# ZrrSkywalker/MonoDETR

Hardware: NVIDIA H100
Metric: images/sec (1280x384, fwd+bwd) (higher is better)
Workload: dtype f32 (BF16x3: error-compensated bf16 tensor-core products, fp32 accumulate)

## Files before the change

### monodetr_b200/csrc/attention.cu

```cuda
#include <cuda_runtime.h>
#include <math.h>
#include <stdint.h>

#include "../../include/monodetr_b200.h"
#include "launch.cuh"
#include "rng.cuh"
#include "tc_common.cuh"

namespace {

using namespace mdb;

constexpr int HD = 32;
constexpr int BR = 64;
constexpr int BC = 64;
constexpr int kTileBytes = BC * HD * 4;
constexpr int ATT_THREADS = 128;

struct AttnParams {
    const float *q, *k, *v;
    const uint8_t* kpm;
    float* out;
    float* lse;
    int B, H, Lq, Lk, ldq, ldk, ldv, ldo;
    float scale;
    float drop_p;
    const unsigned long long* seed;
    unsigned long long site;
    const float *dout, *o;
    float* delta;
    float *dq, *dk, *dv;
    int lddq, lddk, lddv;
};

__device__ __forceinline__ uint32_t f2tf32(float x) {
    uint32_t r;
    asm("cvt.rna.tf32.f32 %0, %1;" : "=r"(r) : "f"(x));
    return r;
}
__device__ __forceinline__ void split_tf32(float x, uint32_t& hi, uint32_t& lo) {
    hi = f2tf32(x);
    lo = f2tf32(x - __uint_as_float(hi));
}
struct AFrag {
    uint32_t hi[4][4];
    uint32_t lo[4][4];
};
__device__ __forceinline__ void load_afrag(AFrag& f, const float* base, int ld, int r0, int nrows, int lane, float mul) {
    const int g = lane >> 2, t = lane & 3;
    const int ra = r0 + g, rb = r0 + g + 8;
    const float* pa = base + (size_t)min(ra, nrows - 1) * ld;
    const float* pb = base + (size_t)min(rb, nrows - 1) * ld;
    const float ma = ra < nrows ? mul : 0.f, mb = rb < nrows ? mul : 0.f;
#pragma unroll
    for (int ks = 0; ks < 4; ++ks) {
        split_tf32(pa[ks * 8 + t] * ma, f.hi[ks][0], f.lo[ks][0]);
        split_tf32(pb[ks * 8 + t] * mb, f.hi[ks][1], f.lo[ks][1]);
        split_tf32(pa[ks * 8 + t + 4] * ma, f.hi[ks][2], f.lo[ks][2]);
        split_tf32(pb[ks * 8 + t + 4] * mb, f.hi[ks][3], f.lo[ks][3]);
    }
}

__device__ __forceinline__ uint32_t nt_off(int r, int c) { return (uint32_t)(r * 128 + ((((c >> 2) ^ (r & 7))) << 4) + (c & 3) * 4); }
__device__ __forceinline__ uint32_t nn_off(int r, int c) {
    const int kk = r & 31, q = kk & 7;
    const int kpos = (kk & ~7) + ((q & 1) ? 4 + (q >> 1) : (q >> 1));
    return (uint32_t)((r >> 5) * 4096 + c * 128 + ((((kpos >> 2) ^ (c & 7))) << 4) + (kpos & 3) * 4);
}

template <int NS>
__device__ __forceinline__ void gemm_nt(float (&c)[8][4], const AFrag& a, uint32_t th, uint32_t tl) {
    float (&d)[32] = reinterpret_cast<float (&)[32]>(c);
#pragma unroll
    for (int i = 0; i < 32; ++i) d[i] = 0.f;
    wgmma_fence();
#pragma unroll
    for (int ks = 0; ks < 4; ++ks) {
        const uint64_t bh = make_wgmma_desc_sw128(th + ks * 32);
        if (NS == 3) {
            const uint64_t bl = make_wgmma_desc_sw128(tl + ks * 32);
            wgmma_tf32_n64(d, a.lo[ks], bh, 1);
            wgmma_tf32_n64(d, a.hi[ks], bl, 1);
        }
        wgmma_tf32_n64(d, a.hi[ks], bh, 1);
    }
    wgmma_commit();
    wgmma_wait_all();
    wgmma_fence_operands(d);
}

template <int NS>
__device__ __forceinline__ void gemm_nn(float (&acc)[4][4], const float (&p)[8][4], uint32_t th, uint32_t tl) {
    float (&d)[16] = reinterpret_cast<float (&)[16]>(acc);
#pragma unroll
    for (int half = 0; half < 2; ++half) {
        uint32_t ah[4][4], al[4][4];
#pragma unroll
        for (int u = 0; u < 4; ++u) {
            const int kt = half * 4 + u;
            split_tf32(p[kt][0], ah[u][0], al[u][0]);
            split_tf32(p[kt][2], ah[u][1], al[u][1]);
            split_tf32(p[kt][1], ah[u][2], al[u][2]);
            split_tf32(p[kt][3], ah[u][3], al[u][3]);
        }
        wgmma_fence();
#pragma unroll
        for (int u = 0; u < 4; ++u) {
            const uint32_t off = half * 4096 + u * 32;
            const uint64_t bh = make_wgmma_desc_sw128(th + off);
            if (NS == 3) {
                const uint64_t bl = make_wgmma_desc_sw128(tl + off);
                wgmma_tf32_n32(d, al[u], bh, 1);
                wgmma_tf32_n32(d, ah[u], bl, 1);
            }
            wgmma_tf32_n32(d, ah[u], bh, 1);
        }
        wgmma_commit();
        wgmma_wait_all();
        wgmma_fence_operands(d);
    }
}

constexpr int STG = BC * HD;
__device__ __forceinline__ void stage_tile(float* stg, const float* base, int ld, int r0, int nrows) {
#pragma unroll
    for (int u = 0; u < 4; ++u) {
        const int i = threadIdx.x + u * ATT_THREADS;
        const int r = i >> 3, c = (i & 7) * 4;
        const bool ok = r0 + r < nrows;
        const float* src = ok ? base + ((size_t)(r0 + r) * ld + c) : base;
        const uint32_t dst = (uint32_t)__cvta_generic_to_shared(stg) + (uint32_t)i * 16u;
        const int nbytes = ok ? 16 : 0;
        asm volatile("cp.async.cg.shared.global [%0], [%1], 16, %2;" ::"r"(dst), "l"(src), "r"(nbytes) : "memory");
    }
}
__device__ __forceinline__ void stage_commit() { asm volatile("cp.async.commit_group;" ::: "memory"); }
__device__ __forceinline__ void stage_wait() { asm volatile("cp.async.wait_all;" ::: "memory"); }
__device__ __forceinline__ void unstage_tile(uint8_t* nt_hi, uint8_t* nt_lo, uint8_t* nn_hi, uint8_t* nn_lo, const float* stg) {
#pragma unroll
    for (int u = 0; u < 4; ++u) {
        const int i = threadIdx.x + u * ATT_THREADS;
        const int r = i >> 3, c = (i & 7) * 4;
        const float4 v = *reinterpret_cast<const float4*>(stg + i * 4);
        uint32_t h[4], l[4];
        split_tf32(v.x, h[0], l[0]); split_tf32(v.y, h[1], l[1]); split_tf32(v.z, h[2], l[2]); split_tf32(v.w, h[3], l[3]);
        if (nt_hi) *reinterpret_cast<uint4*>(nt_hi + nt_off(r, c)) = make_uint4(h[0], h[1], h[2], h[3]);
        if (nt_lo) *reinterpret_cast<uint4*>(nt_lo + nt_off(r, c)) = make_uint4(l[0], l[1], l[2], l[3]);
#pragma unroll
        for (int e = 0; e < 4; ++e) {
            if (nn_hi) *reinterpret_cast<uint32_t*>(nn_hi + nn_off(r, c + e)) = h[e];
            if (nn_lo) *reinterpret_cast<uint32_t*>(nn_lo + nn_off(r, c + e)) = l[e];
        }
    }
}
static_assert(BC * (HD / 4) == 4 * ATT_THREADS, "tile loader mapping");

__device__ __forceinline__ float quad_max(float v) {
    v = fmaxf(v, __shfl_xor_sync(0xffffffffu, v, 1));
    return fmaxf(v, __shfl_xor_sync(0xffffffffu, v, 2));
}
__device__ __forceinline__ float quad_sum(float v) {
    v += __shfl_xor_sync(0xffffffffu, v, 1);
    return v + __shfl_xor_sync(0xffffffffu, v, 2);
}

struct DropCtx {
    uint32_t key, thr;
    float inv_keep;
    bool on;
};
__device__ __forceinline__ DropCtx make_drop(const AttnParams& p, int b, int h) {
    DropCtx d;
    d.on = p.drop_p > 0.f;
    d.inv_keep = 1.f / (1.f - p.drop_p);
    d.thr = mdb::rng_thr16(p.drop_p);
    d.key = 0u;
    if (d.on) d.key = mdb::rng_key32(*p.seed + p.site * 0x9E3779B97F4A7C15ull, (unsigned long long)(b * p.H + h));
    return d;
}
__device__ __forceinline__ float keep_scale(const DropCtx& d, uint32_t row_base, int j) {
    return mdb::rng_keep16(d.key, row_base + (uint32_t)j, d.thr) ? d.inv_keep : 0.f;
}

__device__ __forceinline__ uint32_t fetch_dead(const AttnParams& p, int b, int k0) {
    const int j = k0 + (int)threadIdx.x;
    if (threadIdx.x >= BC) return 0u;
    if (j >= p.Lk) return 1u;
    return (p.kpm && p.kpm[(size_t)b * p.Lk + j]) ? 1u : 0u;
}

__global__ void __launch_bounds__(ATT_THREADS, 3)
attn_fwd_kernel(const AttnParams p) {
    extern __shared__ __align__(1024) uint8_t dyn_smem[];
    uint8_t* sKh = dyn_smem;
    uint8_t* sKl = sKh + kTileBytes;
    uint8_t* sVh = sKl + kTileBytes;
    uint8_t* sVl = sVh + kTileBytes;
    float* gK = reinterpret_cast<float*>(sVl + kTileBytes);
    float* gV = gK + STG;
    uint8_t* sDead = reinterpret_cast<uint8_t*>(gV + STG);
    const int b = blockIdx.z, h = blockIdx.y;
    const int warp = threadIdx.x >> 5, lane = threadIdx.x & 31;
    const int g = lane >> 2, t = lane & 3;
    const int r0 = blockIdx.x * BR + warp * 16;
    const float* qb = p.q + (size_t)b * p.Lq * p.ldq + h * HD;
    const float* kb = p.k + (size_t)b * p.Lk * p.ldk + h * HD;
    const float* vb = p.v + (size_t)b * p.Lk * p.ldv + h * HD;
    const DropCtx drop = make_drop(p, b, h);
    stage_tile(gK, kb, p.ldk, 0, p.Lk);
    stage_tile(gV, vb, p.ldv, 0, p.Lk);
    stage_commit();
    uint32_t ndead = fetch_dead(p, b, 0);
    AFrag qa;
    load_afrag(qa, qb, p.ldq, r0, p.Lq, lane, p.scale);
    float acc[4][4];
#pragma unroll
    for (int i = 0; i < 4; ++i) acc[i][0] = acc[i][1] = acc[i][2] = acc[i][3] = 0.f;
    float m0 = -INFINITY, m1 = -INFINITY, l0 = 0.f, l1 = 0.f;
    const int qi0 = r0 + g, qi1 = r0 + g + 8;
    const uint32_t rb0 = (uint32_t)qi0 * (uint32_t)p.Lk, rb1 = (uint32_t)qi1 * (uint32_t)p.Lk;

    for (int k0 = 0; k0 < p.Lk; k0 += BC) {
        stage_wait();
        __syncthreads();
        unstage_tile(sKh, sKl, nullptr, nullptr, gK);
        unstage_tile(nullptr, nullptr, sVh, sVl, gV);
        if (threadIdx.x < BC) sDead[threadIdx.x] = (uint8_t)ndead;
        mdb::fence_proxy_async_smem();
        __syncthreads();
        if (k0 + BC < p.Lk) {
            stage_tile(gK, kb, p.ldk, k0 + BC, p.Lk);
            stage_tile(gV, vb, p.ldv, k0 + BC, p.Lk);
            stage_commit();
            ndead = fetch_dead(p, b, k0 + BC);
        }
        float s[8][4];
        gemm_nt<3>(s, qa, mdb::smem_u32(sKh), mdb::smem_u32(sKl));
        float mx0 = -INFINITY, mx1 = -INFINITY;
#pragma unroll
        for (int nt = 0; nt < 8; ++nt) {
            const uchar2 dd = *reinterpret_cast<const uchar2*>(&sDead[nt * 8 + 2 * t]);
            if (dd.x) { s[nt][0] = -INFINITY; s[nt][2] = -INFINITY; }
            if (dd.y) { s[nt][1] = -INFINITY; s[nt][3] = -INFINITY; }
            mx0 = fmaxf(mx0, fmaxf(s[nt][0], s[nt][1]));
            mx1 = fmaxf(mx1, fmaxf(s[nt][2], s[nt][3]));
        }
        const float mn0 = fmaxf(m0, quad_max(mx0)), mn1 = fmaxf(m1, quad_max(mx1));
        const float c0 = (mn0 == -INFINITY) ? 1.f : __expf(m0 - mn0), c1 = (mn1 == -INFINITY) ? 1.f : __expf(m1 - mn1);
        l0 *= c0; l1 *= c1;
#pragma unroll
        for (int dn = 0; dn < 4; ++dn) { acc[dn][0] *= c0; acc[dn][1] *= c0; acc[dn][2] *= c1; acc[dn][3] *= c1; }
#pragma unroll
        for (int nt = 0; nt < 8; ++nt) {
#pragma unroll
            for (int e = 0; e < 2; ++e) {
                const int j = k0 + nt * 8 + 2 * t + e;
                float p0 = (mn0 == -INFINITY) ? 0.f : __expf(s[nt][e] - mn0);
                float p1 = (mn1 == -INFINITY) ? 0.f : __expf(s[nt][2 + e] - mn1);
                l0 += p0; l1 += p1;
                if (drop.on) {
                    p0 *= keep_scale(drop, rb0, j);
                    p1 *= keep_scale(drop, rb1, j);
                }
                s[nt][e] = p0; s[nt][2 + e] = p1;
            }
        }
        m0 = mn0; m1 = mn1;
        gemm_nn<3>(acc, s, mdb::smem_u32(sVh), mdb::smem_u32(sVl));
    }
    l0 = quad_sum(l0); l1 = quad_sum(l1);
    const float i0 = l0 > 0.f ? 1.f / l0 : 0.f, i1 = l1 > 0.f ? 1.f / l1 : 0.f;
    float* ob = p.out + (size_t)b * p.Lq * p.ldo + h * HD;
#pragma unroll
    for (int dn = 0; dn < 4; ++dn) {
        if (qi0 < p.Lq) *reinterpret_cast<float2*>(ob + (size_t)qi0 * p.ldo + dn * 8 + 2 * t) = make_float2(acc[dn][0] * i0, acc[dn][1] * i0);
        if (qi1 < p.Lq) *reinterpret_cast<float2*>(ob + (size_t)qi1 * p.ldo + dn * 8 + 2 * t) = make_float2(acc[dn][2] * i1, acc[dn][3] * i1);
    }
    if (t == 0) {
        float* lp = p.lse + ((size_t)b * p.H + h) * p.Lq;
        if (qi0 < p.Lq) lp[qi0] = l0 > 0.f ? m0 + __logf(l0) : -INFINITY;
        if (qi1 < p.Lq) lp[qi1] = l1 > 0.f ? m1 + __logf(l1) : -INFINITY;
    }
}

__global__ void attn_delta_kernel(const AttnParams p) {
    const long long idx = blockIdx.x * (long long)blockDim.x + threadIdx.x;
    const long long n = (long long)p.B * p.Lq * p.H;
    if (idx >= n) return;
    const int h = (int)(idx % p.H);
    const long long bi = idx / p.H;
    const int i = (int)(bi % p.Lq);
    const int b = (int)(bi / p.Lq);
    const float* a = p.dout + (size_t)bi * p.ldo + h * HD;
    const float* o = p.o + (size_t)bi * p.ldo + h * HD;
    float s = 0.f;
#pragma unroll
    for (int d = 0; d < HD; d += 4) {
        const float4 x = *reinterpret_cast<const float4*>(a + d);
        const float4 y = *reinterpret_cast<const float4*>(o + d);
        s += x.x * y.x + x.y * y.y + x.z * y.z + x.w * y.w;
    }
    p.delta[((size_t)b * p.H + h) * p.Lq + i] = s;
}

__global__ void __launch_bounds__(ATT_THREADS, 3)
attn_bwd_dq_kernel(const AttnParams p) {
    extern __shared__ __align__(1024) uint8_t dyn_smem[];
    uint8_t* sKh = dyn_smem;
    uint8_t* sKl = sKh + kTileBytes;
    uint8_t* sKn = sKl + kTileBytes;
    uint8_t* sVh = sKn + kTileBytes;
    float* gK = reinterpret_cast<float*>(sVh + kTileBytes);
    float* gV = gK + STG;
    uint8_t* sDead = reinterpret_cast<uint8_t*>(gV + STG);
    const int b = blockIdx.z, h = blockIdx.y;
    const int warp = threadIdx.x >> 5, lane = threadIdx.x & 31;
    const int g = lane >> 2, t = lane & 3;
    const int r0 = blockIdx.x * BR + warp * 16;
    const float* qb = p.q + (size_t)b * p.Lq * p.ldq + h * HD;
    const float* gb = p.dout + (size_t)b * p.Lq * p.ldo + h * HD;
    const float* kb = p.k + (size_t)b * p.Lk * p.ldk + h * HD;
    const float* vb = p.v + (size_t)b * p.Lk * p.ldv + h * HD;
    const DropCtx drop = make_drop(p, b, h);
    stage_tile(gK, kb, p.ldk, 0, p.Lk);
    stage_tile(gV, vb, p.ldv, 0, p.Lk);
    stage_commit();
    uint32_t ndead = fetch_dead(p, b, 0);
    AFrag qa, ga;
    load_afrag(qa, qb, p.ldq, r0, p.Lq, lane, p.scale);
    load_afrag(ga, gb, p.ldo, r0, p.Lq, lane, 1.f);
    const int qi0 = r0 + g, qi1 = r0 + g + 8;
    const uint32_t rb0 = (uint32_t)qi0 * (uint32_t)p.Lk, rb1 = (uint32_t)qi1 * (uint32_t)p.Lk;
    const size_t st = ((size_t)b * p.H + h) * p.Lq;
    float lse0 = qi0 < p.Lq ? p.lse[st + qi0] : INFINITY, lse1 = qi1 < p.Lq ? p.lse[st + qi1] : INFINITY;
    if (lse0 == -INFINITY) lse0 = INFINITY;
    if (lse1 == -INFINITY) lse1 = INFINITY;
    const float dl0 = qi0 < p.Lq ? p.delta[st + qi0] : 0.f, dl1 = qi1 < p.Lq ? p.delta[st + qi1] : 0.f;
    float acc[4][4];
#pragma unroll
    for (int i = 0; i < 4; ++i) acc[i][0] = acc[i][1] = acc[i][2] = acc[i][3] = 0.f;

    for (int k0 = 0; k0 < p.Lk; k0 += BC) {
        stage_wait();
        __syncthreads();
        unstage_tile(sKh, sKl, sKn, nullptr, gK);
        unstage_tile(sVh, nullptr, nullptr, nullptr, gV);
        if (threadIdx.x < BC) sDead[threadIdx.x] = (uint8_t)ndead;
        mdb::fence_proxy_async_smem();
        __syncthreads();
        if (k0 + BC < p.Lk) {
            stage_tile(gK, kb, p.ldk, k0 + BC, p.Lk);
            stage_tile(gV, vb, p.ldv, k0 + BC, p.Lk);
            stage_commit();
            ndead = fetch_dead(p, b, k0 + BC);
        }
        float s[8][4], dp[8][4];
        gemm_nt<3>(s, qa, mdb::smem_u32(sKh), mdb::smem_u32(sKl));
        gemm_nt<1>(dp, ga, mdb::smem_u32(sVh), 0u);
#pragma unroll
        for (int nt = 0; nt < 8; ++nt) {
            const uchar2 dd = *reinterpret_cast<const uchar2*>(&sDead[nt * 8 + 2 * t]);
#pragma unroll
            for (int e = 0; e < 2; ++e) {
                const int j = k0 + nt * 8 + 2 * t + e;
                const bool dead = e ? dd.y : dd.x;
                float p0 = dead ? 0.f : __expf(s[nt][e] - lse0);
                float p1 = dead ? 0.f : __expf(s[nt][2 + e] - lse1);
                float d0 = dp[nt][e], d1 = dp[nt][2 + e];
                if (drop.on) {
                    d0 *= keep_scale(drop, rb0, j);
                    d1 *= keep_scale(drop, rb1, j);
                }
                s[nt][e] = p0 * (d0 - dl0);
                s[nt][2 + e] = p1 * (d1 - dl1);
            }
        }
        gemm_nn<1>(acc, s, mdb::smem_u32(sKn), 0u);
    }
    float* ob = p.dq + (size_t)b * p.Lq * p.lddq + h * HD;
#pragma unroll
    for (int dn = 0; dn < 4; ++dn) {
        if (qi0 < p.Lq) *reinterpret_cast<float2*>(ob + (size_t)qi0 * p.lddq + dn * 8 + 2 * t) = make_float2(acc[dn][0] * p.scale, acc[dn][1] * p.scale);
        if (qi1 < p.Lq) *reinterpret_cast<float2*>(ob + (size_t)qi1 * p.lddq + dn * 8 + 2 * t) = make_float2(acc[dn][2] * p.scale, acc[dn][3] * p.scale);
    }
}

__global__ void __launch_bounds__(ATT_THREADS, 2)
attn_bwd_dkv_kernel(const AttnParams p) {
    extern __shared__ __align__(1024) uint8_t dyn_smem[];
    uint8_t* sQh = dyn_smem;
    uint8_t* sQl = sQh + kTileBytes;
    uint8_t* sQn = sQl + kTileBytes;
    uint8_t* sGh = sQn + kTileBytes;
    uint8_t* sGn = sGh + kTileBytes;
    float* gQ = reinterpret_cast<float*>(sGn + kTileBytes);
    float* gG = gQ + STG;
    float* sL = gG + STG;
    float* sD = sL + BC;
    const int b = blockIdx.z, h = blockIdx.y;
    const int warp = threadIdx.x >> 5, lane = threadIdx.x & 31;
    const int g = lane >> 2, t = lane & 3;
    const int r0 = blockIdx.x * BR + warp * 16;
    const float* qb = p.q + (size_t)b * p.Lq * p.ldq + h * HD;
    const float* gb = p.dout + (size_t)b * p.Lq * p.ldo + h * HD;
    const float* kb = p.k + (size_t)b * p.Lk * p.ldk + h * HD;
    const float* vb = p.v + (size_t)b * p.Lk * p.ldv + h * HD;
    const DropCtx drop = make_drop(p, b, h);
    const size_t st = ((size_t)b * p.H + h) * p.Lq;
    auto fetch_stats = [&](int q0, float& l, float& d) {
        const int i = q0 + (int)threadIdx.x;
        l = INFINITY; d = 0.f;
        if (threadIdx.x < BC && i < p.Lq) {
            l = p.lse[st + i];
            d = p.delta[st + i];
            if (l == -INFINITY) l = INFINITY;
        }
    };
    float nl, nd;
    stage_tile(gQ, qb, p.ldq, 0, p.Lq);
    stage_tile(gG, gb, p.ldo, 0, p.Lq);
    stage_commit();
    fetch_stats(0, nl, nd);
    AFrag ka, va;
    load_afrag(ka, kb, p.ldk, r0, p.Lk, lane, p.scale);
    load_afrag(va, vb, p.ldv, r0, p.Lk, lane, 1.f);
    const int kj0 = r0 + g, kj1 = r0 + g + 8;
    const bool dead0 = kj0 >= p.Lk || (p.kpm && p.kpm[(size_t)b * p.Lk + min(kj0, p.Lk - 1)]);
    const bool dead1 = kj1 >= p.Lk || (p.kpm && p.kpm[(size_t)b * p.Lk + min(kj1, p.Lk - 1)]);
    float dk[4][4], dv[4][4];
#pragma unroll
    for (int i = 0; i < 4; ++i) {
        dk[i][0] = dk[i][1] = dk[i][2] = dk[i][3] = 0.f;
        dv[i][0] = dv[i][1] = dv[i][2] = dv[i][3] = 0.f;
    }

    for (int q0 = 0; q0 < p.Lq; q0 += BC) {
        stage_wait();
        __syncthreads();
        unstage_tile(sQh, sQl, sQn, nullptr, gQ);
        unstage_tile(sGh, nullptr, sGn, nullptr, gG);
        if (threadIdx.x < BC) { sL[threadIdx.x] = nl; sD[threadIdx.x] = nd; }
        mdb::fence_proxy_async_smem();
        __syncthreads();
        if (q0 + BC < p.Lq) {
            stage_tile(gQ, qb, p.ldq, q0 + BC, p.Lq);
            stage_tile(gG, gb, p.ldo, q0 + BC, p.Lq);
            stage_commit();
            fetch_stats(q0 + BC, nl, nd);
        }
        float s[8][4], dp[8][4];
        gemm_nt<3>(s, ka, mdb::smem_u32(sQh), mdb::smem_u32(sQl));
        gemm_nt<1>(dp, va, mdb::smem_u32(sGh), 0u);
        float pd[8][4];
#pragma unroll
        for (int nt = 0; nt < 8; ++nt) {
            const float2 l2 = *reinterpret_cast<const float2*>(&sL[nt * 8 + 2 * t]);
            const float2 d2 = *reinterpret_cast<const float2*>(&sD[nt * 8 + 2 * t]);
#pragma unroll
            for (int e = 0; e < 2; ++e) {
                const int i = q0 + nt * 8 + 2 * t + e;
                const float lse = e ? l2.y : l2.x, dl = e ? d2.y : d2.x;
                float p0 = dead0 ? 0.f : __expf(s[nt][e] - lse);
                float p1 = dead1 ? 0.f : __expf(s[nt][2 + e] - lse);
                float d0 = dp[nt][e], d1 = dp[nt][2 + e];
                float w0 = p0, w1 = p1;
                if (drop.on) {
                    const uint32_t rb = (uint32_t)i * (uint32_t)p.Lk;
                    const float k0s = keep_scale(drop, rb, kj0), k1s = keep_scale(drop, rb, kj1);
                    w0 *= k0s; w1 *= k1s; d0 *= k0s; d1 *= k1s;
                }
                pd[nt][e] = w0; pd[nt][2 + e] = w1;
                s[nt][e] = p0 * (d0 - dl);
                s[nt][2 + e] = p1 * (d1 - dl);
            }
        }
        gemm_nn<1>(dv, pd, mdb::smem_u32(sGn), 0u);
        gemm_nn<1>(dk, s, mdb::smem_u32(sQn), 0u);
    }
    float* dkb = p.dk + (size_t)b * p.Lk * p.lddk + h * HD;
    float* dvb = p.dv + (size_t)b * p.Lk * p.lddv + h * HD;
#pragma unroll
    for (int dn = 0; dn < 4; ++dn) {
        if (kj0 < p.Lk) {
            *reinterpret_cast<float2*>(dkb + (size_t)kj0 * p.lddk + dn * 8 + 2 * t) = make_float2(dk[dn][0] * p.scale, dk[dn][1] * p.scale);
            *reinterpret_cast<float2*>(dvb + (size_t)kj0 * p.lddv + dn * 8 + 2 * t) = make_float2(dv[dn][0], dv[dn][1]);
        }
        if (kj1 < p.Lk) {
            *reinterpret_cast<float2*>(dkb + (size_t)kj1 * p.lddk + dn * 8 + 2 * t) = make_float2(dk[dn][2] * p.scale, dk[dn][3] * p.scale);
            *reinterpret_cast<float2*>(dvb + (size_t)kj1 * p.lddv + dn * 8 + 2 * t) = make_float2(dv[dn][2], dv[dn][3]);
        }
    }
}

constexpr int kFwdSmem = 4 * kTileBytes + 2 * STG * 4 + BC;
constexpr int kDqSmem = 4 * kTileBytes + 2 * STG * 4 + BC;
constexpr int kDkvSmem = 5 * kTileBytes + 2 * STG * 4 + 2 * BC * 4;

int check(const AttnParams& p) {
    if (p.B <= 0 || p.H <= 0 || p.Lq <= 0 || p.Lk <= 0) return MDB_EINVAL;
    if ((p.ldq | p.ldk | p.ldv | p.ldo) % 4) return MDB_EINVAL;
    if (p.drop_p < 0.f || p.drop_p >= 1.f) return MDB_EINVAL;
    if (p.drop_p > 0.f && !p.seed) return MDB_EINVAL;
    if (p.H > 65535 || p.B > 65535) return MDB_EUNSUPPORTED;
    if ((unsigned long long)p.Lq * (unsigned long long)p.Lk >= (1ull << 32)) return MDB_EUNSUPPORTED;
    return 0;
}

}

extern "C" {

int mdb_attention_forward_f32(const float* q, const float* k, const float* v, const unsigned char* key_padding_mask,
                              float* out, float* lse, int B, int H, int Lq, int Lk, int head_dim, int ldq, int ldk,
                              int ldv, int ldo, float drop_p, const unsigned long long* seed, unsigned long long site,
                              void* stream) {
    if (head_dim != HD) return MDB_EUNSUPPORTED;
    if (!q || !k || !v || !out || !lse) return MDB_EINVAL;
    AttnParams p{};
    p.q = q; p.k = k; p.v = v; p.kpm = key_padding_mask; p.out = out; p.lse = lse;
    p.B = B; p.H = H; p.Lq = Lq; p.Lk = Lk; p.ldq = ldq; p.ldk = ldk; p.ldv = ldv; p.ldo = ldo;
    p.scale = 1.f / sqrtf((float)HD); p.drop_p = drop_p; p.seed = seed; p.site = site;
    int rc = check(p);
    if (rc) return rc;
    dim3 grid((Lq + BR - 1) / BR, H, B);
    const cudaError_t e = set_max_dynamic_smem(attn_fwd_kernel, kFwdSmem);
    if (e != cudaSuccess) return (int)e;
    attn_fwd_kernel<<<grid, ATT_THREADS, kFwdSmem, static_cast<cudaStream_t>(stream)>>>(p);
    return (int)cudaGetLastError();
}

int mdb_attention_backward_f32(const float* q, const float* k, const float* v, const unsigned char* key_padding_mask,
                               const float* out, const float* lse, const float* dout, float* delta_ws, float* dq,
                               float* dk, float* dv, int B, int H, int Lq, int Lk, int head_dim, int ldq, int ldk, int ldv,
                               int ldo, int lddq, int lddk, int lddv, float drop_p, const unsigned long long* seed,
                               unsigned long long site, void* stream_) {
    if (head_dim != HD) return MDB_EUNSUPPORTED;
    if (!q || !k || !v || !out || !lse || !dout || !delta_ws || !dq || !dk || !dv) return MDB_EINVAL;
    cudaStream_t stream = static_cast<cudaStream_t>(stream_);
    AttnParams p{};
    p.q = q; p.k = k; p.v = v; p.kpm = key_padding_mask; p.lse = const_cast<float*>(lse);
    p.B = B; p.H = H; p.Lq = Lq; p.Lk = Lk; p.ldq = ldq; p.ldk = ldk; p.ldv = ldv; p.ldo = ldo;
    p.scale = 1.f / sqrtf((float)HD); p.drop_p = drop_p; p.seed = seed; p.site = site;
    p.dout = dout; p.o = out; p.delta = delta_ws; p.dq = dq; p.dk = dk; p.dv = dv;
    p.lddq = lddq; p.lddk = lddk; p.lddv = lddv;
    int rc = check(p);
    if (rc) return rc;
    if ((lddq | lddk | lddv) % 4) return MDB_EINVAL;
    const long long n = (long long)B * Lq * H;
    attn_delta_kernel<<<(unsigned)((n + 255) / 256), 256, 0, stream>>>(p);
    cudaError_t e = set_max_dynamic_smem(attn_bwd_dq_kernel, kDqSmem);
    if (e == cudaSuccess) e = set_max_dynamic_smem(attn_bwd_dkv_kernel, kDkvSmem);
    if (e != cudaSuccess) return (int)e;
    attn_bwd_dq_kernel<<<dim3((Lq + BR - 1) / BR, H, B), ATT_THREADS, kDqSmem, stream>>>(p);
    attn_bwd_dkv_kernel<<<dim3((Lk + BR - 1) / BR, H, B), ATT_THREADS, kDkvSmem, stream>>>(p);
    return (int)cudaGetLastError();
}

}
```

Before: 173.5.

## Share streamed K/V and Q/dO tiles across multiple warpgroups in attention backward

The dq and dkv backward kernels can now run several warpgroups per CTA (three for dq when the grid is large enough, two for dkv). Each streamed tile is converted and split into hi/lo once and reused by every warpgroup, and double-buffered shared tiles remove one barrier per iteration. The two QK/dO GEMMs now issue back to back before a single wait. Dropout masks are generated two at a time from one hash, and the dkv kernel maps key rows in adjacent pairs so the pairs line up. This cuts global loads and split work per output row but lowers occupancy, leaves idle warpgroups in tail CTAs, and changes the dropout RNG layout.

```diff
diff --git a/monodetr_b200/csrc/attention.cu b/monodetr_b200/csrc/attention.cu
--- a/monodetr_b200/csrc/attention.cu
+++ b/monodetr_b200/csrc/attention.cu
@@ -15,7 +15,7 @@
 constexpr int BR = 64;
 constexpr int BC = 64;
 constexpr int kTileBytes = BC * HD * 4;
-constexpr int ATT_THREADS = 128;
+constexpr int WG_THREADS = 128;
 
 struct AttnParams {
     const float *q, *k, *v;
@@ -46,9 +46,10 @@
     uint32_t hi[4][4];
     uint32_t lo[4][4];
 };
+template <bool PAIRED = false>
 __device__ __forceinline__ void load_afrag(AFrag& f, const float* base, int ld, int r0, int nrows, int lane, float mul) {
     const int g = lane >> 2, t = lane & 3;
-    const int ra = r0 + g, rb = r0 + g + 8;
+    const int ra = PAIRED ? r0 + 2 * g : r0 + g, rb = PAIRED ? r0 + 2 * g + 1 : r0 + g + 8;
     const float* pa = base + (size_t)min(ra, nrows - 1) * ld;
     const float* pb = base + (size_t)min(rb, nrows - 1) * ld;
     const float ma = ra < nrows ? mul : 0.f, mb = rb < nrows ? mul : 0.f;
@@ -68,7 +69,7 @@
     return (uint32_t)((r >> 5) * 4096 + c * 128 + ((((kpos >> 2) ^ (c & 7))) << 4) + (kpos & 3) * 4);
 }
 
-template <int NS>
+template <int NS, bool WAIT = true>
 __device__ __forceinline__ void gemm_nt(float (&c)[8][4], const AFrag& a, uint32_t th, uint32_t tl) {
     float (&d)[32] = reinterpret_cast<float (&)[32]>(c);
 #pragma unroll
@@ -85,8 +86,10 @@
         wgmma_tf32_n64(d, a.hi[ks], bh, 1);
     }
     wgmma_commit();
-    wgmma_wait_all();
-    wgmma_fence_operands(d);
+    if (WAIT) {
+        wgmma_wait_all();
+        wgmma_fence_operands(d);
+    }
 }
 
 template <int NS>
@@ -122,10 +125,13 @@
 }
 
 constexpr int STG = BC * HD;
+constexpr int kChunks = STG / 4;
+template <int NT>
 __device__ __forceinline__ void stage_tile(float* stg, const float* base, int ld, int r0, int nrows) {
 #pragma unroll
-    for (int u = 0; u < 4; ++u) {
-        const int i = threadIdx.x + u * ATT_THREADS;
+    for (int u = 0; u < (kChunks + NT - 1) / NT; ++u) {
+        const int i = threadIdx.x + u * NT;
+        if (kChunks % NT != 0 && i >= kChunks) break;
         const int r = i >> 3, c = (i & 7) * 4;
         const bool ok = r0 + r < nrows;
         const float* src = ok ? base + ((size_t)(r0 + r) * ld + c) : base;
@@ -136,10 +142,12 @@
 }
 __device__ __forceinline__ void stage_commit() { asm volatile("cp.async.commit_group;" ::: "memory"); }
 __device__ __forceinline__ void stage_wait() { asm volatile("cp.async.wait_all;" ::: "memory"); }
+template <int NT>
 __device__ __forceinline__ void unstage_tile(uint8_t* nt_hi, uint8_t* nt_lo, uint8_t* nn_hi, uint8_t* nn_lo, const float* stg) {
 #pragma unroll
-    for (int u = 0; u < 4; ++u) {
-        const int i = threadIdx.x + u * ATT_THREADS;
+    for (int u = 0; u < (kChunks + NT - 1) / NT; ++u) {
+        const int i = threadIdx.x + u * NT;
+        if (kChunks % NT != 0 && i >= kChunks) break;
         const int r = i >> 3, c = (i & 7) * 4;
         const float4 v = *reinterpret_cast<const float4*>(stg + i * 4);
         uint32_t h[4], l[4];
@@ -153,7 +161,13 @@
         }
     }
 }
-static_assert(BC * (HD / 4) == 4 * ATT_THREADS, "tile loader mapping");
+static_assert(BC <= WG_THREADS, "per-row flags of the streamed tile are fetched by the first BC threads");
+
+template <int NWG> struct CtaShape {
+    static constexpr int kThreads = NWG * WG_THREADS;
+    static constexpr int kRows = NWG * BR;
+    static constexpr int kBufs = NWG > 1 ? 2 : 1;
+};
 
 __device__ __forceinline__ float quad_max(float v) {
     v = fmaxf(v, __shfl_xor_sync(0xffffffffu, v, 1));
@@ -181,6 +195,19 @@
 __device__ __forceinline__ float keep_scale(const DropCtx& d, uint32_t row_base, int j) {
     return mdb::rng_keep16(d.key, row_base + (uint32_t)j, d.thr) ? d.inv_keep : 0.f;
 }
+__device__ __forceinline__ void keep_scale_pair(const DropCtx& d, uint32_t idx, float& s0, float& s1) {
+    const uint32_t h = mdb::rng_pair32(d.key, idx >> 1);
+    s0 = h >= (d.thr << 16) ? d.inv_keep : 0.f;
+    s1 = mdb::rng_pair32_odd(h) >= (d.thr << 16) ? d.inv_keep : 0.f;
+}
+__device__ __forceinline__ void keep_scale2(const DropCtx& d, uint32_t idx, bool paired, float& s0, float& s1) {
+    if (paired) {
+        keep_scale_pair(d, idx, s0, s1);
+    } else {
+        s0 = keep_scale(d, idx, 0);
+        s1 = keep_scale(d, idx + 1u, 0);
+    }
+}
 
 __device__ __forceinline__ uint32_t fetch_dead(const AttnParams& p, int b, int k0) {
     const int j = k0 + (int)threadIdx.x;
@@ -189,7 +216,8 @@
     return (p.kpm && p.kpm[(size_t)b * p.Lk + j]) ? 1u : 0u;
 }
 
-__global__ void __launch_bounds__(ATT_THREADS, 3)
+constexpr int kFwdSmem = 4 * kTileBytes + 2 * STG * 4 + BC;
+__global__ void __launch_bounds__(WG_THREADS, 3)
 attn_fwd_kernel(const AttnParams p) {
     extern __shared__ __align__(1024) uint8_t dyn_smem[];
     uint8_t* sKh = dyn_smem;
@@ -207,8 +235,8 @@
     const float* kb = p.k + (size_t)b * p.Lk * p.ldk + h * HD;
     const float* vb = p.v + (size_t)b * p.Lk * p.ldv + h * HD;
     const DropCtx drop = make_drop(p, b, h);
-    stage_tile(gK, kb, p.ldk, 0, p.Lk);
-    stage_tile(gV, vb, p.ldv, 0, p.Lk);
+    stage_tile<WG_THREADS>(gK, kb, p.ldk, 0, p.Lk);
+    stage_tile<WG_THREADS>(gV, vb, p.ldv, 0, p.Lk);
     stage_commit();
     uint32_t ndead = fetch_dead(p, b, 0);
     AFrag qa;
@@ -219,18 +247,19 @@
     float m0 = -INFINITY, m1 = -INFINITY, l0 = 0.f, l1 = 0.f;
     const int qi0 = r0 + g, qi1 = r0 + g + 8;
     const uint32_t rb0 = (uint32_t)qi0 * (uint32_t)p.Lk, rb1 = (uint32_t)qi1 * (uint32_t)p.Lk;
+    const bool pair0 = !(rb0 & 1u), pair1 = !(rb1 & 1u);
 
     for (int k0 = 0; k0 < p.Lk; k0 += BC) {
         stage_wait();
         __syncthreads();
-        unstage_tile(sKh, sKl, nullptr, nullptr, gK);
-        unstage_tile(nullptr, nullptr, sVh, sVl, gV);
+        unstage_tile<WG_THREADS>(sKh, sKl, nullptr, nullptr, gK);
+        unstage_tile<WG_THREADS>(nullptr, nullptr, sVh, sVl, gV);
         if (threadIdx.x < BC) sDead[threadIdx.x] = (uint8_t)ndead;
         mdb::fence_proxy_async_smem();
         __syncthreads();
         if (k0 + BC < p.Lk) {
-            stage_tile(gK, kb, p.ldk, k0 + BC, p.Lk);
-            stage_tile(gV, vb, p.ldv, k0 + BC, p.Lk);
+            stage_tile<WG_THREADS>(gK, kb, p.ldk, k0 + BC, p.Lk);
+            stage_tile<WG_THREADS>(gV, vb, p.ldv, k0 + BC, p.Lk);
             stage_commit();
             ndead = fetch_dead(p, b, k0 + BC);
         }
@@ -252,15 +281,20 @@
         for (int dn = 0; dn < 4; ++dn) { acc[dn][0] *= c0; acc[dn][1] *= c0; acc[dn][2] *= c1; acc[dn][3] *= c1; }
 #pragma unroll
         for (int nt = 0; nt < 8; ++nt) {
+            float ka[2], kb[2];
+            if (drop.on) {
+                const uint32_t j = (uint32_t)(k0 + nt * 8 + 2 * t);
+                keep_scale2(drop, rb0 + j, pair0, ka[0], ka[1]);
+                keep_scale2(drop, rb1 + j, pair1, kb[0], kb[1]);
+            }
 #pragma unroll
             for (int e = 0; e < 2; ++e) {
-                const int j = k0 + nt * 8 + 2 * t + e;
                 float p0 = (mn0 == -INFINITY) ? 0.f : __expf(s[nt][e] - mn0);
                 float p1 = (mn1 == -INFINITY) ? 0.f : __expf(s[nt][2 + e] - mn1);
                 l0 += p0; l1 += p1;
                 if (drop.on) {
-                    p0 *= keep_scale(drop, rb0, j);
-                    p1 *= keep_scale(drop, rb1, j);
+                    p0 *= ka[e];
+                    p1 *= kb[e];
                 }
                 s[nt][e] = p0; s[nt][2 + e] = p1;
             }
@@ -303,27 +337,29 @@
     p.delta[((size_t)b * p.H + h) * p.Lq + i] = s;
 }
 
-__global__ void __launch_bounds__(ATT_THREADS, 3)
+constexpr int kDqBuf = 4 * kTileBytes + 1024;
+template <int NWG>
+constexpr int dq_smem() { return CtaShape<NWG>::kBufs * kDqBuf + 2 * STG * 4; }
+
+template <int NWG>
+__global__ void __launch_bounds__(CtaShape<NWG>::kThreads, NWG == 1 ? 3 : 1)
 attn_bwd_dq_kernel(const AttnParams p) {
+    using S = CtaShape<NWG>;
     extern __shared__ __align__(1024) uint8_t dyn_smem[];
-    uint8_t* sKh = dyn_smem;
-    uint8_t* sKl = sKh + kTileBytes;
-    uint8_t* sKn = sKl + kTileBytes;
-    uint8_t* sVh = sKn + kTileBytes;
-    float* gK = reinterpret_cast<float*>(sVh + kTileBytes);
+    float* gK = reinterpret_cast<float*>(dyn_smem + S::kBufs * kDqBuf);
     float* gV = gK + STG;
-    uint8_t* sDead = reinterpret_cast<uint8_t*>(gV + STG);
     const int b = blockIdx.z, h = blockIdx.y;
     const int warp = threadIdx.x >> 5, lane = threadIdx.x & 31;
     const int g = lane >> 2, t = lane & 3;
-    const int r0 = blockIdx.x * BR + warp * 16;
+    const int r0 = blockIdx.x * S::kRows + warp * 16;
+    const bool active = NWG == 1 || blockIdx.x * S::kRows + (warp >> 2) * BR < p.Lq;
     const float* qb = p.q + (size_t)b * p.Lq * p.ldq + h * HD;
     const float* gb = p.dout + (size_t)b * p.Lq * p.ldo + h * HD;
     const float* kb = p.k + (size_t)b * p.Lk * p.ldk + h * HD;
     const float* vb = p.v + (size_t)b * p.Lk * p.ldv + h * HD;
     const DropCtx drop = make_drop(p, b, h);
-    stage_tile(gK, kb, p.ldk, 0, p.Lk);
-    stage_tile(gV, vb, p.ldv, 0, p.Lk);
+    stage_tile<S::kThreads>(gK, kb, p.ldk, 0, p.Lk);
+    stage_tile<S::kThreads>(gV, vb, p.ldv, 0, p.Lk);
     stage_commit();
     uint32_t ndead = fetch_dead(p, b, 0);
     AFrag qa, ga;
@@ -331,6 +367,7 @@
     load_afrag(ga, gb, p.ldo, r0, p.Lq, lane, 1.f);
     const int qi0 = r0 + g, qi1 = r0 + g + 8;
     const uint32_t rb0 = (uint32_t)qi0 * (uint32_t)p.Lk, rb1 = (uint32_t)qi1 * (uint32_t)p.Lk;
+    const bool pair0 = !(rb0 & 1u), pair1 = !(rb1 & 1u);
     const size_t st = ((size_t)b * p.H + h) * p.Lq;
     float lse0 = qi0 < p.Lq ? p.lse[st + qi0] : INFINITY, lse1 = qi1 < p.Lq ? p.lse[st + qi1] : INFINITY;
     if (lse0 == -INFINITY) lse0 = INFINITY;
@@ -340,36 +377,50 @@
 #pragma unroll
     for (int i = 0; i < 4; ++i) acc[i][0] = acc[i][1] = acc[i][2] = acc[i][3] = 0.f;
 
-    for (int k0 = 0; k0 < p.Lk; k0 += BC) {
+    for (int k0 = 0, it = 0; k0 < p.Lk; k0 += BC, ++it) {
+        uint8_t* sKh = dyn_smem + (S::kBufs > 1 ? (it & 1) : 0) * kDqBuf;
+        uint8_t* sKl = sKh + kTileBytes;
+        uint8_t* sKn = sKl + kTileBytes;
+        uint8_t* sVh = sKn + kTileBytes;
+        uint8_t* sDead = sVh + kTileBytes;
         stage_wait();
-        __syncthreads();
-        unstage_tile(sKh, sKl, sKn, nullptr, gK);
-        unstage_tile(sVh, nullptr, nullptr, nullptr, gV);
+        if (S::kBufs == 1) __syncthreads();
+        unstage_tile<S::kThreads>(sKh, sKl, sKn, nullptr, gK);
+        unstage_tile<S::kThreads>(sVh, nullptr, nullptr, nullptr, gV);
         if (threadIdx.x < BC) sDead[threadIdx.x] = (uint8_t)ndead;
         mdb::fence_proxy_async_smem();
         __syncthreads();
         if (k0 + BC < p.Lk) {
-            stage_tile(gK, kb, p.ldk, k0 + BC, p.Lk);
-            stage_tile(gV, vb, p.ldv, k0 + BC, p.Lk);
+            stage_tile<S::kThreads>(gK, kb, p.ldk, k0 + BC, p.Lk);
+            stage_tile<S::kThreads>(gV, vb, p.ldv, k0 + BC, p.Lk);
             stage_commit();
             ndead = fetch_dead(p, b, k0 + BC);
         }
+        if (!active) continue;
         float s[8][4], dp[8][4];
-        gemm_nt<3>(s, qa, mdb::smem_u32(sKh), mdb::smem_u32(sKl));
-        gemm_nt<1>(dp, ga, mdb::smem_u32(sVh), 0u);
+        gemm_nt<3, false>(s, qa, mdb::smem_u32(sKh), mdb::smem_u32(sKl));
+        gemm_nt<1, false>(dp, ga, mdb::smem_u32(sVh), 0u);
+        wgmma_wait_all();
+        wgmma_fence_operands(reinterpret_cast<float (&)[32]>(s));
+        wgmma_fence_operands(reinterpret_cast<float (&)[32]>(dp));
 #pragma unroll
         for (int nt = 0; nt < 8; ++nt) {
             const uchar2 dd = *reinterpret_cast<const uchar2*>(&sDead[nt * 8 + 2 * t]);
+            float ka[2], kb[2];
+            if (drop.on) {
+                const uint32_t j = (uint32_t)(k0 + nt * 8 + 2 * t);
+                keep_scale2(drop, rb0 + j, pair0, ka[0], ka[1]);
+                keep_scale2(drop, rb1 + j, pair1, kb[0], kb[1]);
+            }
 #pragma unroll
             for (int e = 0; e < 2; ++e) {
-                const int j = k0 + nt * 8 + 2 * t + e;
                 const bool dead = e ? dd.y : dd.x;
                 float p0 = dead ? 0.f : __expf(s[nt][e] - lse0);
                 float p1 = dead ? 0.f : __expf(s[nt][2 + e] - lse1);
                 float d0 = dp[nt][e], d1 = dp[nt][2 + e];
                 if (drop.on) {
-                    d0 *= keep_scale(drop, rb0, j);
-                    d1 *= keep_scale(drop, rb1, j);
+                    d0 *= ka[e];
+                    d1 *= kb[e];
                 }
                 s[nt][e] = p0 * (d0 - dl0);
                 s[nt][2 + e] = p1 * (d1 - dl1);
@@ -377,6 +428,7 @@
         }
         gemm_nn<1>(acc, s, mdb::smem_u32(sKn), 0u);
     }
+    if (!active) return;
     float* ob = p.dq + (size_t)b * p.Lq * p.lddq + h * HD;
 #pragma unroll
     for (int dn = 0; dn < 4; ++dn) {
@@ -385,22 +437,22 @@
     }
 }
 
-__global__ void __launch_bounds__(ATT_THREADS, 2)
+constexpr int kDkvBuf = 5 * kTileBytes + 1024;
+template <int NWG>
+constexpr int dkv_smem() { return CtaShape<NWG>::kBufs * kDkvBuf + 2 * STG * 4; }
+
+template <int NWG>
+__global__ void __launch_bounds__(CtaShape<NWG>::kThreads, NWG == 1 ? 2 : 1)
 attn_bwd_dkv_kernel(const AttnParams p) {
+    using S = CtaShape<NWG>;
     extern __shared__ __align__(1024) uint8_t dyn_smem[];
-    uint8_t* sQh = dyn_smem;
-    uint8_t* sQl = sQh + kTileBytes;
-    uint8_t* sQn = sQl + kTileBytes;
-    uint8_t* sGh = sQn + kTileBytes;
-    uint8_t* sGn = sGh + kTileBytes;
-    float* gQ = reinterpret_cast<float*>(sGn + kTileBytes);
+    float* gQ = reinterpret_cast<float*>(dyn_smem + S::kBufs * kDkvBuf);
     float* gG = gQ + STG;
-    float* sL = gG + STG;
-    float* sD = sL + BC;
     const int b = blockIdx.z, h = blockIdx.y;
     const int warp = threadIdx.x >> 5, lane = threadIdx.x & 31;
     const int g = lane >> 2, t = lane & 3;
-    const int r0 = blockIdx.x * BR + warp * 16;
+    const int r0 = blockIdx.x * S::kRows + warp * 16;
+    const bool active = NWG == 1 || blockIdx.x * S::kRows + (warp >> 2) * BR < p.Lk;
     const float* qb = p.q + (size_t)b * p.Lq * p.ldq + h * HD;
     const float* gb = p.dout + (size_t)b * p.Lq * p.ldo + h * HD;
     const float* kb = p.k + (size_t)b * p.Lk * p.ldk + h * HD;
@@ -417,14 +469,14 @@
         }
     };
     float nl, nd;
-    stage_tile(gQ, qb, p.ldq, 0, p.Lq);
-    stage_tile(gG, gb, p.ldo, 0, p.Lq);
+    stage_tile<S::kThreads>(gQ, qb, p.ldq, 0, p.Lq);
+    stage_tile<S::kThreads>(gG, gb, p.ldo, 0, p.Lq);
     stage_commit();
     fetch_stats(0, nl, nd);
     AFrag ka, va;
-    load_afrag(ka, kb, p.ldk, r0, p.Lk, lane, p.scale);
-    load_afrag(va, vb, p.ldv, r0, p.Lk, lane, 1.f);
-    const int kj0 = r0 + g, kj1 = r0 + g + 8;
+    load_afrag<true>(ka, kb, p.ldk, r0, p.Lk, lane, p.scale);
+    load_afrag<true>(va, vb, p.ldv, r0, p.Lk, lane, 1.f);
+    const int kj0 = r0 + 2 * g, kj1 = kj0 + 1;
     const bool dead0 = kj0 >= p.Lk || (p.kpm && p.kpm[(size_t)b * p.Lk + min(kj0, p.Lk - 1)]);
     const bool dead1 = kj1 >= p.Lk || (p.kpm && p.kpm[(size_t)b * p.Lk + min(kj1, p.Lk - 1)]);
     float dk[4][4], dv[4][4];
@@ -434,23 +486,34 @@
         dv[i][0] = dv[i][1] = dv[i][2] = dv[i][3] = 0.f;
     }
 
-    for (int q0 = 0; q0 < p.Lq; q0 += BC) {
+    for (int q0 = 0, it = 0; q0 < p.Lq; q0 += BC, ++it) {
+        uint8_t* sQh = dyn_smem + (S::kBufs > 1 ? (it & 1) : 0) * kDkvBuf;
+        uint8_t* sQl = sQh + kTileBytes;
+        uint8_t* sQn = sQl + kTileBytes;
+        uint8_t* sGh = sQn + kTileBytes;
+        uint8_t* sGn = sGh + kTileBytes;
+        float* sL = reinterpret_cast<float*>(sGn + kTileBytes);
+        float* sD = sL + BC;
         stage_wait();
-        __syncthreads();
-        unstage_tile(sQh, sQl, sQn, nullptr, gQ);
-        unstage_tile(sGh, nullptr, sGn, nullptr, gG);
+        if (S::kBufs == 1) __syncthreads();
+        unstage_tile<S::kThreads>(sQh, sQl, sQn, nullptr, gQ);
+        unstage_tile<S::kThreads>(sGh, nullptr, sGn, nullptr, gG);
         if (threadIdx.x < BC) { sL[threadIdx.x] = nl; sD[threadIdx.x] = nd; }
         mdb::fence_proxy_async_smem();
         __syncthreads();
         if (q0 + BC < p.Lq) {
-            stage_tile(gQ, qb, p.ldq, q0 + BC, p.Lq);
-            stage_tile(gG, gb, p.ldo, q0 + BC, p.Lq);
+            stage_tile<S::kThreads>(gQ, qb, p.ldq, q0 + BC, p.Lq);
+            stage_tile<S::kThreads>(gG, gb, p.ldo, q0 + BC, p.Lq);
             stage_commit();
             fetch_stats(q0 + BC, nl, nd);
         }
+        if (!active) continue;
         float s[8][4], dp[8][4];
-        gemm_nt<3>(s, ka, mdb::smem_u32(sQh), mdb::smem_u32(sQl));
-        gemm_nt<1>(dp, va, mdb::smem_u32(sGh), 0u);
+        gemm_nt<3, false>(s, ka, mdb::smem_u32(sQh), mdb::smem_u32(sQl));
+        gemm_nt<1, false>(dp, va, mdb::smem_u32(sGh), 0u);
+        wgmma_wait_all();
+        wgmma_fence_operands(reinterpret_cast<float (&)[32]>(s));
+        wgmma_fence_operands(reinterpret_cast<float (&)[32]>(dp));
         float pd[8][4];
 #pragma unroll
         for (int nt = 0; nt < 8; ++nt) {
@@ -466,7 +529,8 @@
                 float w0 = p0, w1 = p1;
                 if (drop.on) {
                     const uint32_t rb = (uint32_t)i * (uint32_t)p.Lk;
-                    const float k0s = keep_scale(drop, rb, kj0), k1s = keep_scale(drop, rb, kj1);
+                    float k0s, k1s;
+                    keep_scale2(drop, rb + (uint32_t)kj0, !(rb & 1u), k0s, k1s);
                     w0 *= k0s; w1 *= k1s; d0 *= k0s; d1 *= k1s;
                 }
                 pd[nt][e] = w0; pd[nt][2 + e] = w1;
@@ -477,6 +541,7 @@
         gemm_nn<1>(dv, pd, mdb::smem_u32(sGn), 0u);
         gemm_nn<1>(dk, s, mdb::smem_u32(sQn), 0u);
     }
+    if (!active) return;
     float* dkb = p.dk + (size_t)b * p.Lk * p.lddk + h * HD;
     float* dvb = p.dv + (size_t)b * p.Lk * p.lddv + h * HD;
 #pragma unroll
@@ -491,10 +556,6 @@
         }
     }
 }
-
-constexpr int kFwdSmem = 4 * kTileBytes + 2 * STG * 4 + BC;
-constexpr int kDqSmem = 4 * kTileBytes + 2 * STG * 4 + BC;
-constexpr int kDkvSmem = 5 * kTileBytes + 2 * STG * 4 + 2 * BC * 4;
 
 int check(const AttnParams& p) {
     if (p.B <= 0 || p.H <= 0 || p.Lq <= 0 || p.Lk <= 0) return MDB_EINVAL;
@@ -504,6 +565,32 @@
     if (p.H > 65535 || p.B > 65535) return MDB_EUNSUPPORTED;
     if ((unsigned long long)p.Lq * (unsigned long long)p.Lk >= (1ull << 32)) return MDB_EUNSUPPORTED;
     return 0;
+}
+
+bool dq_three_warpgroups(const AttnParams& p) {
+    if (p.Lq <= BR) return false;
+    int dev = 0, sms = 0;
+    if (cudaGetDevice(&dev) != cudaSuccess || cudaDeviceGetAttribute(&sms, cudaDevAttrMultiProcessorCount, dev) != cudaSuccess)
+        return false;
+    const long long ctas = (long long)((p.Lq + CtaShape<3>::kRows - 1) / CtaShape<3>::kRows) * p.H * p.B;
+    return ctas >= 4LL * sms;
+}
+
+template <int NWG>
+cudaError_t launch_dq(const AttnParams& p, cudaStream_t stream) {
+    const cudaError_t e = set_max_dynamic_smem(attn_bwd_dq_kernel<NWG>, dq_smem<NWG>());
+    if (e != cudaSuccess) return e;
+    attn_bwd_dq_kernel<NWG><<<dim3((p.Lq + CtaShape<NWG>::kRows - 1) / CtaShape<NWG>::kRows, p.H, p.B),
+                              CtaShape<NWG>::kThreads, dq_smem<NWG>(), stream>>>(p);
+    return cudaGetLastError();
+}
+template <int NWG>
+cudaError_t launch_dkv(const AttnParams& p, cudaStream_t stream) {
+    const cudaError_t e = set_max_dynamic_smem(attn_bwd_dkv_kernel<NWG>, dkv_smem<NWG>());
+    if (e != cudaSuccess) return e;
+    attn_bwd_dkv_kernel<NWG><<<dim3((p.Lk + CtaShape<NWG>::kRows - 1) / CtaShape<NWG>::kRows, p.H, p.B),
+                               CtaShape<NWG>::kThreads, dkv_smem<NWG>(), stream>>>(p);
+    return cudaGetLastError();
 }
 
 }
@@ -522,10 +609,10 @@
     p.scale = 1.f / sqrtf((float)HD); p.drop_p = drop_p; p.seed = seed; p.site = site;
     int rc = check(p);
     if (rc) return rc;
-    dim3 grid((Lq + BR - 1) / BR, H, B);
+    cudaStream_t s = static_cast<cudaStream_t>(stream);
     const cudaError_t e = set_max_dynamic_smem(attn_fwd_kernel, kFwdSmem);
     if (e != cudaSuccess) return (int)e;
-    attn_fwd_kernel<<<grid, ATT_THREADS, kFwdSmem, static_cast<cudaStream_t>(stream)>>>(p);
+    attn_fwd_kernel<<<dim3((Lq + BR - 1) / BR, H, B), WG_THREADS, kFwdSmem, s>>>(p);
     return (int)cudaGetLastError();
 }
 
@@ -548,12 +635,9 @@
     if ((lddq | lddk | lddv) % 4) return MDB_EINVAL;
     const long long n = (long long)B * Lq * H;
     attn_delta_kernel<<<(unsigned)((n + 255) / 256), 256, 0, stream>>>(p);
-    cudaError_t e = set_max_dynamic_smem(attn_bwd_dq_kernel, kDqSmem);
-    if (e == cudaSuccess) e = set_max_dynamic_smem(attn_bwd_dkv_kernel, kDkvSmem);
-    if (e != cudaSuccess) return (int)e;
-    attn_bwd_dq_kernel<<<dim3((Lq + BR - 1) / BR, H, B), ATT_THREADS, kDqSmem, stream>>>(p);
-    attn_bwd_dkv_kernel<<<dim3((Lk + BR - 1) / BR, H, B), ATT_THREADS, kDkvSmem, stream>>>(p);
-    return (int)cudaGetLastError();
-}
-
-}
+    cudaError_t e = dq_three_warpgroups(p) ? launch_dq<3>(p, stream) : launch_dq<1>(p, stream);
+    if (e == cudaSuccess) e = Lk > BR ? launch_dkv<2>(p, stream) : launch_dkv<1>(p, stream);
+    return (int)e;
+}
+
+}
```

New measurement: 174.2 (median of 6 runs). No clear change (+0.4%).
